# Restream/reindexer

Hardware: NVIDIA H100
Metric: KNN QPS @ recall@10 (10Mx768, k=10) + HBM GB/s vs roofline (higher is better)
Workload: dtype f32

## Files before the change

### reindexer_b200/csrc/index.cu

```cuda
#include <cuda_runtime.h>

#include <cub/device/device_scan.cuh>
#include <cub/device/device_segmented_radix_sort.cuh>

#include <algorithm>
#include <atomic>
#include <cstdio>
#include <cstdlib>
#include <cstring>
#include <limits>
#include <memory>
#include <mutex>
#include <new>
#include <string>
#include <unordered_map>
#include <unordered_set>
#include <vector>

#include "../../include/rxgpu.h"
#include "internal.h"
#include "../host/knn_select.h"
#include "knn_scan.cuh"
#include "knn_tc.cuh"
#include "ivf_select.cuh"
// ... 138 lines not shown
		a.queries = d_queries + size_t(q0) * ix->dim;
		a.nq = std::min<uint32_t>(qt, nq - q0);
		for (uint32_t round = 0; round < rounds; ++round) {
			a.k1 = std::min(kr, k1 - round * kr);
			a.floor_keys = round ? ws.d_floor.p : nullptr;
			cudaEvent_t e0 = nullptr, e1 = nullptr;
			if (g_profile.load(std::memory_order_relaxed)) {
				RX_CUDA(cudaEventCreate(&e0));
				RX_CUDA(cudaEventCreate(&e1));
				RX_CUDA(cudaEventRecord(e0, st));
			}
			RX_CUDA(launchScan(ix, qt, a, &grid, st));
			if (e0) {
				RX_CUDA(cudaEventRecord(e1, st));
				g_prof_events.emplace_back(e0, e1);
			}
			MergeArgs m{};
			m.lists = ws.d_lists.p;
			m.labels = ix->d_labels;
			m.out_dist = d_out_dist;
			m.out_idx = d_out_idx;
			m.out_label = d_out_label;
			m.out_count = d_out_count;
			m.floor_out = rounds > 1 ? ws.d_floor.p : nullptr;
			m.nlists = grid;
			m.qt = qt;
			m.k1 = a.k1;
			m.q_offset = q0;
			m.out_stride = k1;
			m.out_offset = round * kr;
			m.mode = mode;
			m.neg_zero = ix->metric != RXGPU_L2;
			knn_merge_lists<<<a.nq, 256, 0, st>>>(m);
			RX_CUDA(cudaGetLastError());
			g_stats.launches += 2;
			g_stats.passes += 1;
		}
	}
	g_stats.query_tile = uint32_t(qt);
	const uint64_t perPass = uint64_t(nrows) * ix->dim * 4 + (ix->metric == RXGPU_COS ? uint64_t(nrows) * 4 : 0) +
							 uint64_t(qt) * ix->dim * 4 + uint64_t(qt) * kr * 12;
	g_stats.algorithmic_bytes += perPass * ((nq + qt - 1) / qt) * rounds;
	return 0;
}

using EncodeTiledFn = CUresult (*)(CUtensorMap*, CUtensorMapDataType, cuuint32_t, void*, const cuuint64_t*, const cuuint64_t*,
								   const cuuint32_t*, const cuuint32_t*, CUtensorMapInterleave, CUtensorMapSwizzle, CUtensorMapL2promotion,
								   CUtensorMapFloatOOBfill);
EncodeTiledFn encodeTiled() {
	static EncodeTiledFn fn = [] {
		void* p = nullptr;
		cudaDriverEntryPointQueryResult q;
		if (cudaGetDriverEntryPoint("cuTensorMapEncodeTiled", &p, cudaEnableDefault, &q) != cudaSuccess || q != cudaDriverEntryPointSuccess) {
			cudaGetLastError();
			return EncodeTiledFn(nullptr);
		}
		return reinterpret_cast<EncodeTiledFn>(p);
	}();
	return fn;
}
int makeCodeMap(CUtensorMap* m, void* base, uint64_t pitchBytes, uint64_t rows, uint32_t boxRows) {
	const cuuint64_t gdim[2] = {pitchBytes, rows};
	const cuuint64_t gstr[1] = {pitchBytes};
	const cuuint32_t box[2] = {uint32_t(kTcChunkK), boxRows};
	const cuuint32_t estr[2] = {1, 1};
	const CUresult r = encodeTiled()(m, CU_TENSOR_MAP_DATA_TYPE_UINT8, 2, base, gdim, gstr, box, estr, CU_TENSOR_MAP_INTERLEAVE_NONE,
									  CU_TENSOR_MAP_SWIZZLE_128B, CU_TENSOR_MAP_L2_PROMOTION_L2_256B, CU_TENSOR_MAP_FLOAT_OOB_FILL_NONE);
	if (r != CUDA_SUCCESS) {
		return fail(RXGPU_ERR_SYSTEM, "rxgpu: cuTensorMapEncodeTiled failed (" + std::to_string(int(r)) + ")");
	}
	return 0;
}

constexpr size_t kTcSmemLimit = 227 * 1024;
uint32_t tcCandCap(uint32_t k1) { return std::max<uint32_t>(4096u, 256u * k1); }
uint32_t tcRangeCap(uint64_t max_out) { return uint32_t(std::max<uint64_t>(4096u, 2 * std::min<uint64_t>(max_out, 1u << 17))); }
constexpr uint32_t kStageRatio = 4;
constexpr uint32_t kStageSeedPerK1 = 2;
constexpr uint32_t kStageCapPerK1 = 64;
uint32_t stageSeedRows(uint32_t k1) { return kStageSeedPerK1 * k1; }
uint32_t stageCandCap(uint32_t k1) { return std::min<uint32_t>(1u << 18, std::max<uint32_t>(4096u, kStageCapPerK1 * k1)); }

using TcKernel = void (*)(const CUtensorMap, const TcArgs);
TcKernel tcKernel(uint32_t nqb, uint32_t cluster) {
	static const TcKernel table[4][2] = {{knn_tc_filter<32, 1>, knn_tc_filter<32, 2>},
										 {knn_tc_filter<64, 1>, knn_tc_filter<64, 2>},
										 {knn_tc_filter<96, 1>, knn_tc_filter<96, 2>},
										 {knn_tc_filter<128, 1>, knn_tc_filter<128, 2>}};
	return table[nqb / 32 - 1][cluster == 2 ? 1 : 0];
}
std::atomic<int> g_tc_diag{0};
unsigned long long* g_tc_diag_buf = nullptr;
TcKernel tcDiagKernel(int mode) {
	static const TcKernel table[4] = {knn_tc_filter<128, 1, kTcDiagStamps>, knn_tc_filter<128, 1, kTcDiagNoRare>,
									  knn_tc_filter<128, 1, kTcDiagNoFetch>, knn_tc_filter<128, 1, kTcDiagNoTest>};
	return table[mode - 1];
}

uint32_t tcQueryBlock(uint32_t nq, uint32_t kchunks) {
	uint32_t nqb = std::min<uint32_t>(kTcMaxNq, (nq + 31u) & ~31u);
	while (nqb >= 32 && tc_smem_bytes(nqb, kchunks) > kTcSmemLimit) {
		nqb -= 32;
	}
	if (nqb < 32) {
		return 0;
	}
	const uint32_t blocks = (nq + nqb - 1) / nqb;
	return std::min(nqb, (((nq + blocks - 1) / blocks) + 31u) & ~31u);
}

bool tcServes(const rxgpu_index* ix, uint32_t nq) {
	if (ix->tc_mode == 2 || !encodeTiled()) {
		return false;
	}
	if (tcQueryBlock(nq, (ix->dim + kTcChunkK - 1) / kTcChunkK) == 0) {
		return false;
	}
	if (ix->dim > 2048) {
		return false;
	}
	return ix->tc_mode == 1 || (nq >= 64 && ix->size >= 100000);
}
bool tcEligible(const rxgpu_index* ix, uint32_t nq, uint32_t k1, int mode) {
	return mode == kModeTopK && k1 <= kTcStagedMaxK1 && tcServes(ix, nq);
}

int ensureShadow(const rxgpu_index* ix, cudaStream_t st) {
	std::lock_guard<std::mutex> lck(ix->tc_mtx);
	const uint32_t pitchQ = (ix->dim + kTcChunkK - 1) / kTcChunkK * kTcChunkK;
	if (!ix->d_shadow) {
		const size_t cap = (size_t(ix->capacity ? ix->capacity : 1) + kTcTileRows - 1) / kTcTileRows * kTcTileRows;
		RX_CUDA(cudaMalloc(&ix->d_shadow, cap * pitchQ));
		RX_CUDA(cudaMalloc(reinterpret_cast<void**>(&ix->d_rowc), cap * sizeof(float4)));
		ix->pitch_q = pitchQ;
		ix->shadow_version = ~0ull;
		ix->shadow_dirty_all = true;
		ix->shadow_dirty.clear();
	}
	if (ix->shadow_version != ix->version) {
		auto convert = [&](uint32_t b, uint32_t e) {
			const unsigned blocks = unsigned((uint64_t(e - b) * 32 + 255) / 256);
			tc_convert_rows<<<blocks, 256, 0, st>>>(ix->d_rows, ix->pitch, ix->dim, b, e, static_cast<unsigned char*>(ix->d_shadow),
													pitchQ / kTcChunkK, ix->metric == RXGPU_COS ? ix->d_norms : nullptr, ix->d_rowc);
		};
		if (ix->shadow_dirty_all) {
			if (ix->size) {
				convert(0, uint32_t(ix->size));
			}
		} else {
			for (const auto& r : ix->shadow_dirty) {
				const uint32_t e = uint32_t(std::min<uint64_t>(r.second, ix->size));
				if (r.first < e) {
					convert(r.first, e);
				}
			}
		}
		ix->shadow_dirty_all = false;
		ix->shadow_dirty.clear();
		const uint64_t padded = (ix->size + kTcTileRows - 1) / kTcTileRows * kTcTileRows;
		RX_CUDA(cudaMemsetAsync(ix->d_rowc + ix->size, 0, size_t(padded - ix->size) * sizeof(float4), st));
		RX_CUDA(cudaGetLastError());
		RX_CUDA(cudaStreamSynchronize(st));
		ix->shadow_version = ix->version;
		g_stats.launches += 1;
	}
	return 0;
}

struct TcBatch {
	uint32_t nq, nqb, cluster, ngroups, nqPad, kchunks, stages, queueSlots;
	int diag;
	size_t smem;
	int resident;
	TcKernel kfn;
	CUtensorMap mapQ;
};

int tcPrepare(const rxgpu_index* ix, Workspace& ws, cudaStream_t st, const float* d_queries, uint32_t nq, uint32_t candCap, TcBatch& b) {
	if (int rc = ensureShadow(ix, st)) {
		return rc;
	}
	const uint32_t pitchQ = ix->pitch_q, kchunks = pitchQ / kTcChunkK;
	const uint32_t nqb = tcQueryBlock(nq, kchunks);
	const uint32_t ntiles = uint32_t((ix->size + kTcTileRows - 1) / kTcTileRows);
	const uint32_t clusterMax = ix->tc_cluster_max ? ix->tc_cluster_max : 1u;
	const uint32_t cluster = clusterMax >= 2 && nq > nqb && ntiles >= 2 ? 2u : 1u;
	const uint32_t ngroups = ((nq + nqb - 1) / nqb + cluster - 1) / cluster;
	const uint32_t nqPad = ngroups * cluster * nqb;
	RX_CUDA(ws.d_qcodes.ensure(size_t(nqPad) * pitchQ));
	RX_CUDA(ws.d_qc.ensure(nqPad));
	RX_CUDA(ws.d_qf.ensure(size_t(nqPad) * pitchQ));
	RX_CUDA(ws.d_tau.ensure(nqPad));
	RX_CUDA(ws.d_cand_count.ensure(nqPad));
	RX_CUDA(ws.d_cand_rows.ensure(size_t(nqPad) * candCap));
	RX_CUDA(ws.h_cand_count.ensure(nqPad));
	tc_prepare_queries<<<(nqPad * 32 + 255) / 256, 256, 0, st>>>(d_queries, nq, nqPad, ix->dim, pitchQ, ws.d_qcodes.p, ws.d_qc.p,
																 ws.d_qf.p);
	g_stats.launches += 1;
	RX_CUDA(cudaGetLastError());
	if (int rc = makeCodeMap(&b.mapQ, ws.d_qcodes.p, pitchQ, nqPad, nqb)) {
		return rc;
	}
	b.kfn = tcKernel(nqb, cluster);
	b.stages = tc_ring_stages(nqb, kchunks, kTcSmemLimit);
	b.queueSlots = tc_queue_slots(nqb, kchunks, b.stages, kTcSmemLimit);
	b.smem = tc_smem_bytes(nqb, kchunks, b.stages) + tc_queue_bytes(b.queueSlots);
	if (b.stages == 0 || b.queueSlots == 0) {
		return fail(RXGPU_ERR_SYSTEM, "rxgpu: no room for the tensor-core filter's candidate queues");
	}
	b.diag = g_tc_diag.load();
	if (const int diag = b.diag) {
		if (nqb != 128 || cluster != 1) {
			return fail(RXGPU_ERR_PARAMS, "rxgpu: the diagnostic filter instantiations take query blocks of 128 and single CTAs");
		}
		b.kfn = tcDiagKernel(diag);
	}
	RX_CUDA(raiseSmemCeilingOnce(b.kfn, ix->device, int(kTcSmemLimit)));
	cudaLaunchConfig_t cfg{};
	cfg.gridDim = dim3(unsigned(ix->sm_count) / cluster * cluster);
	cfg.blockDim = dim3(kTcThreads);
	cfg.dynamicSmemBytes = b.smem;
	cudaLaunchAttribute attr[1];
	attr[0].id = cudaLaunchAttributeClusterDimension;
	attr[0].val.clusterDim.x = cluster;
	attr[0].val.clusterDim.y = 1;
	attr[0].val.clusterDim.z = 1;
	cfg.attrs = attr;
	cfg.numAttrs = 1;
	b.resident = 0;
	RX_CUDA(cudaOccupancyMaxActiveClusters(&b.resident, b.kfn, &cfg));
	if (b.resident < 1) {
		return fail(RXGPU_ERR_SYSTEM, "rxgpu: tensor-core filter kernel cannot be made resident");
	}
	b.nq = nq;
	b.nqb = nqb;
	b.cluster = cluster;
	b.ngroups = ngroups;
	b.nqPad = nqPad;
	b.kchunks = kchunks;
	return 0;
}

int tcLaunch(const rxgpu_index* ix, Workspace& ws, cudaStream_t st, const TcBatch& b, uint32_t k1, uint32_t candCap, uint32_t nrows, bool fixedTau) {
	const uint32_t nq = b.nq, nqb = b.nqb, cluster = b.cluster, ngroups = b.ngroups, kchunks = b.kchunks, pitchQ = ix->pitch_q;
	const uint32_t ntiles = (nrows + kTcTileRows - 1) / kTcTileRows;
	const int resident = b.resident;
	const TcKernel kfn = b.kfn;
	const CUtensorMap mapQ = b.mapQ;
	RX_CUDA(cudaMemsetAsync(ws.d_cand_count.p, 0, size_t(b.nqPad) * 4, st));
	RX_CUDA(cudaGetLastError());
	cudaLaunchConfig_t cfg{};
	cfg.blockDim = dim3(kTcThreads);
	cfg.dynamicSmemBytes = b.smem;
	cfg.stream = st;
	cudaLaunchAttribute attr[1];
	attr[0].id = cudaLaunchAttributeClusterDimension;
	attr[0].val.clusterDim.x = cluster;
	attr[0].val.clusterDim.y = 1;
	attr[0].val.clusterDim.z = 1;
	cfg.attrs = attr;
	cfg.numAttrs = 1;
	TcArgs a{};
	a.shadow = static_cast<const unsigned char*>(ix->d_shadow);
	a.rowc = ix->d_rowc;
	a.qc = ws.d_qc.p;
	a.tau = ws.d_tau.p;
	a.ub_list = fixedTau ? nullptr : ws.d_ub_list.p;
	a.ub_lock = fixedTau ? nullptr : ws.d_ub_lock.p;
	a.init_rows = fixedTau ? UINT32_MAX : uint32_t(std::min<uint64_t>(ix->size, kTcInitRows));
	a.rows = ix->d_rows;
	a.norm_coefs = ix->metric == RXGPU_COS ? ix->d_norms : nullptr;
	a.qf = ws.d_qf.p;
	a.pitch = ix->pitch;
	a.cand_rows = ws.d_cand_rows.p;
	a.cand_count = ws.d_cand_count.p;
	a.cand_cap = candCap;
	a.n = nrows;
	a.dim = ix->dim;
	a.kchunks = kchunks;
	a.nq_total = nq;
	a.k1 = k1;
	a.metric = ix->metric;
	a.queue_slots = b.queueSlots;
	a.stages = b.stages;
	a.diag = g_tc_diag_buf;
	for (uint32_t g0 = 0; g0 < ngroups;) {
		const uint32_t groups = std::min<uint32_t>(ngroups - g0, uint32_t(resident));
		const uint32_t walkers = uint32_t(std::min<uint64_t>(uint32_t(resident) / groups, ntiles));
		cfg.gridDim = dim3(groups * walkers * cluster);
		a.q0 = g0 * cluster * nqb;
		a.groups = groups;
		cudaEvent_t e0 = nullptr, e1 = nullptr;
		if (g_profile.load(std::memory_order_relaxed)) {
			RX_CUDA(cudaEventCreate(&e0));
			RX_CUDA(cudaEventCreate(&e1));
			RX_CUDA(cudaEventRecord(e0, st));
		}
		RX_CUDA(cudaLaunchKernelEx(&cfg, kfn, mapQ, a));
// ... 612 lines not shown
			return fail(RXGPU_ERR_LOGIC, "The number of elements exceeds the specified limit\n");
		}
	} catch (const std::bad_alloc&) {
		return fail(RXGPU_ERR_SYSTEM, "rxgpu: out of host memory");
	}
	return 0;
}

int rxgpu_index_upsert(rxgpu_index* ix, uint64_t label, const float* vec) { return rxgpu_index_upsert_batch(ix, 1, &label, vec); }

int rxgpu_index_remove(rxgpu_index* ix, uint64_t label) {
	if (int rc = checkIndex(ix)) {
		return rc;
	}
	const uint32_t cur = ix->dict.find(label);
	if (cur == LabelMap::kNotFound) {
		return 0;
	}
	ix->dict.erase(label);
	ix->version++;
	const uint64_t last = ix->size - 1;
	if (cur != last) {
		ix->touchRows(cur, uint64_t(cur) + 1);
		const uint64_t lastLabel = ix->h_labels[last];
		ix->dict.put(lastLabel, cur);
		ix->h_labels[cur] = lastLabel;
		RX_CUDA(cudaMemcpyAsync(ix->d_rows + size_t(cur) * ix->pitch, ix->d_rows + size_t(last) * ix->pitch, ix->pitch * sizeof(float),
								cudaMemcpyDeviceToDevice, ix->stream));
		RX_CUDA(cudaMemcpyAsync(ix->d_labels + cur, ix->d_labels + last, sizeof(uint64_t), cudaMemcpyDeviceToDevice, ix->stream));
		if (ix->d_norms) {
			RX_CUDA(cudaMemcpyAsync(ix->d_norms + cur, ix->d_norms + last, sizeof(float), cudaMemcpyDeviceToDevice, ix->stream));
		}
		if (ix->flags & RXGPU_FLAG_HOST_MIRROR) {
			std::memcpy(ix->h_rows.data() + size_t(cur) * ix->dim, ix->h_rows.data() + size_t(last) * ix->dim, ix->dim * sizeof(float));
		}
		RX_CUDA(cudaStreamSynchronize(ix->stream));
	}
	ix->h_labels.pop_back();
	ix->size--;
	return 0;
}

int rxgpu_index_get(const rxgpu_index* ix, uint64_t label, const float** host_row) {
	if (!ix || !host_row) {
		return fail(RXGPU_ERR_PARAMS, "rxgpu: null handle");
	}
	const uint32_t idx = ix->dict.find(label);
	if (idx == LabelMap::kNotFound) {
		return fail(RXGPU_ERR_NOT_FOUND, "Label not found");
	}
	if (ix->flags & RXGPU_FLAG_HOST_MIRROR) {
		*host_row = ix->h_rows.data() + size_t(idx) * ix->dim;
		return 0;
	}
	RX_CUDA(cudaSetDevice(ix->device));
	g_row_scratch.resize(ix->dim);
	RX_CUDA(cudaMemcpy(g_row_scratch.data(), ix->d_rows + size_t(idx) * ix->pitch, ix->dim * sizeof(float), cudaMemcpyDeviceToHost));
	*host_row = g_row_scratch.data();
	return 0;
}

uint64_t rxgpu_index_size(const rxgpu_index* ix) { return ix ? ix->size : 0; }
uint64_t rxgpu_index_capacity(const rxgpu_index* ix) { return ix ? ix->capacity : 0; }
uint64_t rxgpu_index_element_size(const rxgpu_index* ix) { return ix ? uint64_t(ix->dim) * 4 + 8 : 0; }
uint64_t rxgpu_index_device_bytes(const rxgpu_index* ix) {
	if (!ix) {
		return 0;
	}
	const uint64_t cap = ix->capacity ? ix->capacity : 1;
	return cap * ix->pitch * 4 + cap * 8 + (ix->d_norms ? cap * 4 : 0);
}
uint32_t rxgpu_index_dim(const rxgpu_index* ix) { return ix ? ix->dim : 0; }
int rxgpu_index_metric(const rxgpu_index* ix) { return ix ? ix->metric : -1; }
int rxgpu_index_device(const rxgpu_index* ix) { return ix ? ix->device : -1; }

int rxgpu_set_query_tile(rxgpu_index* ix, uint32_t qt) {
	if (!ix) {
		return fail(RXGPU_ERR_PARAMS, "rxgpu: null handle");
	}
	ix->qt_override = qt;
	return 0;
}
int rxgpu_set_tensor_core_filter(rxgpu_index* ix, int mode) {
	if (!ix || mode < 0 || mode > 4) {
		return fail(RXGPU_ERR_PARAMS, "rxgpu: tensor-core filter mode must be 0..4");
	}
	ix->tc_mode = uint32_t(mode >= 3 ? 1 : mode);
	ix->tc_cluster_max = mode == 4 ? 2u : 0u;
	return 0;
}
int rxgpu_tc_diag(int mode, void* d_counters) {
	if (mode < 0 || mode > kTcDiagNoTest || (mode && !d_counters)) {
		return fail(RXGPU_ERR_PARAMS, "rxgpu: diagnostic filter mode must be 0..4, with a counter buffer");
	}
	const char* env = std::getenv("RXGPU_TC_DIAG");
	if (mode && !(env && std::strcmp(env, "1") == 0)) {
		return fail(RXGPU_ERR_LOGIC, "rxgpu: diagnostic filter instantiations are enabled only with RXGPU_TC_DIAG=1 in the environment");
	}
	g_tc_diag_buf = static_cast<unsigned long long*>(d_counters);
	g_tc_diag.store(mode);
	return 0;
}
int rxgpu_set_profile(int on) {
	g_profile.store(on ? 1 : 0);
	return 0;
}
void rxgpu_last_search_stats(rxgpu_search_stats* out) {
	if (out) {
		*out = g_stats;
	}
}

int rxgpu_search_knn_device(const rxgpu_index* ix, uint32_t nq, const float* d_queries, uint32_t k1, float* d_out_dist,
							uint32_t* d_out_idx, uint64_t* d_out_label, uint32_t* d_out_count, void* stream) {
	if (int rc = checkIndex(ix)) {
		return rc;
	}
	g_stats = rxgpu_search_stats{};
	if (nq == 0) {
		return 0;
	}
	if (k1 == 0 || k1 > kMaxSearchK1) {
		return fail(RXGPU_ERR_PARAMS, "rxgpu: k must be in [1, 65535]");
	}
	WsLease lease(ix);
	Workspace& ws = *lease.ws;
	cudaStream_t st = stream ? static_cast<cudaStream_t>(stream) : ix->stream;
	if (ix->size == 0) {
		RX_CUDA(cudaMemsetAsync(d_out_count, 0, nq * sizeof(uint32_t), st));
		RX_CUDA(cudaStreamSynchronize(st));
		return 0;
	}
	if (int rc = scanTopK(ix, ws, st, d_queries, nq, k1, kModeTopK, 0.f, d_out_dist, d_out_idx, d_out_label, d_out_count)) {
		return rc;
	}
	RX_CUDA(cudaStreamSynchronize(st));
	collectProfile();
	return 0;
}

int rxgpu_search_tie_rows_device(const rxgpu_index* ix, const float* d_query, float dstar, uint32_t k, float* d_out_dist,
								 uint32_t* d_out_idx, uint64_t* d_out_label, uint32_t* d_out_count, void* stream) {
	if (int rc = checkIndex(ix)) {
		return rc;
	}
	if (k == 0 || k > kMaxSearchK1) {
		return fail(RXGPU_ERR_PARAMS, "rxgpu: k must be in [1, 65535]");
	}
	WsLease lease(ix);
	cudaStream_t st = stream ? static_cast<cudaStream_t>(stream) : ix->stream;
	if (ix->size == 0) {
		RX_CUDA(cudaMemsetAsync(d_out_count, 0, sizeof(uint32_t), st));
		RX_CUDA(cudaStreamSynchronize(st));
		return 0;
	}
	if (int rc = scanTopK(ix, *lease.ws, st, d_query, 1, k, kModeTieRows, dstar, d_out_dist, d_out_idx, d_out_label, d_out_count)) {
		return rc;
	}
	RX_CUDA(cudaStreamSynchronize(st));
	g_stats.tie_replays += 1;
	return 0;
}

int rxgpu_merge_shards(uint32_t nshards, uint32_t nq, uint32_t k, uint32_t k1, const float* dist, const uint32_t* idx,
					   const uint64_t* label, const uint32_t* count, const uint64_t* shard_base, float* out_dist, uint64_t* out_gidx,
					   uint64_t* out_label, uint32_t* out_count, uint8_t* need_tie) {
	if (!dist || !idx || !label || !count || !shard_base || !out_dist || !out_gidx || !out_label || !out_count || !need_tie) {
		return fail(RXGPU_ERR_PARAMS, "rxgpu: null argument");
	}
	try {
		std::vector<Hit> all;
// ... 1484 lines not shown
```

### reindexer_b200/csrc/knn_tc.cuh

```cuda
#pragma once
#include <cuda.h>

#include <type_traits>

#include "common.cuh"
#include "knn_scan.cuh"

namespace rxgpu {

constexpr int kTcThreads = 512;
constexpr int kTcConsumers = 3;
constexpr int kTcTileRows = 128;
constexpr int kTcChunkK = 128;
constexpr int kTcStages = 12;
constexpr int kTcStagesMin = 8;
constexpr int kTcBlockBytes = 64 * kTcChunkK;
constexpr uint32_t kTcMaxNq = 128;
constexpr uint32_t kTcMaxK1 = 128;
constexpr float kTcL2Eps = 1e-5f;

struct TcArgs {
	const unsigned char* shadow;
	const float4* rowc;
	const float4* qc;
// ... 1 lines not shown
	float* ub_list;
	unsigned int* ub_lock;
	uint32_t init_rows;
	const float* rows;
	const float* norm_coefs;
	const float* qf;
	uint32_t pitch;
	uint32_t* cand_rows;
	unsigned int* cand_count;
	uint32_t cand_cap;
	uint32_t n;
	uint32_t dim;
	uint32_t kchunks;
	uint32_t nq_total;
	uint32_t q0;
	uint32_t groups;
	uint32_t k1;
	int metric;
	uint32_t queue_slots;
	uint32_t stages;
	unsigned long long* diag;
};

constexpr int kTcDiagStamps = 1;
constexpr int kTcDiagNoRare = 2;
constexpr int kTcDiagNoFetch = 3;
constexpr int kTcDiagNoTest = 4;
constexpr uint32_t kTcDiagSlots = 64;
constexpr uint32_t kTcDiagWalk = 8192;
constexpr uint32_t kTcDiagMarkEvery = 64;
enum : uint32_t {
	kTcDgFull,
	kTcDgMma,
	kTcDgDrain,
	kTcDgBar1,
	kTcDgTest,
	kTcDgAppend,
	kTcDgTurn,
	kTcDgBar2,
	kTcDgTile,
	kTcDgBlocks,
	kTcDgHits,
	kTcDgQueueWait,
	kTcDgPerWg,
	kTcDgEmpty = kTcConsumers * kTcDgPerWg,
	kTcDgProd = kTcDgEmpty + 1,
	kTcDgRescored = kTcDgProd + 1,
	kTcDgInserts,
	kTcDgRescoreCycles,
};
static_assert(kTcDgRescoreCycles < kTcDiagSlots, "diagnostic counters fit their slots");

__host__ __device__ inline size_t tc_smem_bytes(uint32_t nq_block, uint32_t kchunks, uint32_t stages = kTcStages) {
	return 1024  + size_t(nq_block) * kchunks * 128 + size_t(stages) * kTcBlockBytes + 256  +
		   size_t(nq_block) * (16  + kTcConsumers * (4 + 8) ) + 64;
}

__device__ __forceinline__ uint32_t smem_u32(const void* p) { return uint32_t(__cvta_generic_to_shared(p)); }
__device__ __forceinline__ void mbar_init(uint64_t* bar, uint32_t count) {
	asm volatile("mbarrier.init.shared::cta.b64 [%0], %1;" ::"r"(smem_u32(bar)), "r"(count));
}
__device__ __forceinline__ void mbar_expect_tx(uint64_t* bar, uint32_t bytes) {
	asm volatile("mbarrier.arrive.expect_tx.shared::cta.b64 _, [%0], %1;" ::"r"(smem_u32(bar)), "r"(bytes) : "memory");
}
__device__ __forceinline__ void mbar_arrive(uint64_t* bar) {
	asm volatile("mbarrier.arrive.shared::cta.b64 _, [%0];" ::"r"(smem_u32(bar)) : "memory");
}
__device__ __forceinline__ void mbar_wait(uint64_t* bar, uint32_t parity) {
	asm volatile(
		"{\n"
		".reg .pred p;\n"
		"WAIT_%=:\n"
		"mbarrier.try_wait.parity.shared::cta.b64 p, [%0], %1;\n"
		"@p bra DONE_%=;\n"
		"bra WAIT_%=;\n"
		"DONE_%=:\n"
		"}\n" ::"r"(smem_u32(bar)),
		"r"(parity)
		: "memory");
}
__device__ __forceinline__ void mbar_arrive_cluster(uint64_t* bar, uint32_t cta) {
	uint32_t remote;
	asm volatile("mapa.shared::cluster.u32 %0, %1, %2;" : "=r"(remote) : "r"(smem_u32(bar)), "r"(cta));
	asm volatile("mbarrier.arrive.release.cluster.shared::cluster.b64 _, [%0];" ::"r"(remote) : "memory");
}
__device__ __forceinline__ void tma_load_2d(void* dst, const CUtensorMap* map, uint64_t* bar, int32_t x, int32_t y) {
	asm volatile("cp.async.bulk.tensor.2d.shared::cluster.global.tile.mbarrier::complete_tx::bytes [%0], [%1, {%3, %4}], [%2];" ::"r"(
					 smem_u32(dst)),
				 "l"(map), "r"(smem_u32(bar)), "r"(x), "r"(y)
				 : "memory");
}
__device__ __forceinline__ void bulk_load(void* dst, const void* src, uint32_t bytes, uint64_t* bar) {
	asm volatile("cp.async.bulk.shared::cluster.global.mbarrier::complete_tx::bytes [%0], [%1], %2, [%3];" ::"r"(smem_u32(dst)), "l"(src),
				 "r"(bytes), "r"(smem_u32(bar))
				 : "memory");
}
__device__ __forceinline__ void bulk_load_mc(void* dst, const void* src, uint32_t bytes, uint64_t* bar, uint16_t mask) {
	asm volatile("cp.async.bulk.shared::cluster.global.mbarrier::complete_tx::bytes.multicast::cluster [%0], [%1], %2, [%3], %4;" ::"r"(
					 smem_u32(dst)),
				 "l"(src), "r"(bytes), "r"(smem_u32(bar)), "h"(mask)
				 : "memory");
}
__device__ __forceinline__ bool elect_one_sync() {
	uint32_t p;
	asm volatile(
		"{\n"
		".reg .pred P;\n"
		"elect.sync _|P, 0xffffffff;\n"
		"selp.u32 %0, 1, 0, P;\n"
		"}\n"
		: "=r"(p));
	return p != 0;
}
__device__ __forceinline__ uint32_t cluster_ctarank() {
	uint32_t r;
	asm volatile("mov.u32 %0, %%cluster_ctarank;" : "=r"(r));
	return r;
}
__device__ __forceinline__ void cluster_sync_all() {
	asm volatile("barrier.cluster.arrive.release.aligned;" ::: "memory");
	asm volatile("barrier.cluster.wait.acquire.aligned;" ::: "memory");
}
__device__ __forceinline__ uint64_t wgmma_desc_sw128(uint32_t smem_addr) {
	uint64_t d = 0;
	d |= uint64_t((smem_addr & 0x3FFFFu) >> 4);
	d |= uint64_t(1) << 16;
	d |= uint64_t(1024 >> 4) << 32;
	d |= uint64_t(1) << 62;
	return d;
}
__device__ __forceinline__ void wgmma_fence() { asm volatile("wgmma.fence.sync.aligned;" ::: "memory"); }
__device__ __forceinline__ void wgmma_commit() { asm volatile("wgmma.commit_group.sync.aligned;" ::: "memory"); }
template <int N>
__device__ __forceinline__ void wgmma_wait() {
	asm volatile("wgmma.wait_group.sync.aligned %0;" ::"n"(N) : "memory");
}
__device__ __forceinline__ void wgmma_m64n32k32(int (&d)[16], uint64_t adesc, uint64_t bdesc, uint32_t accumulate) {
	asm volatile(
		"{\n"
		".reg .pred p;\n"
		"setp.ne.b32 p, %18, 0;\n"
		"wgmma.mma_async.sync.aligned.m64n32k32.s32.s8.s8 "
		"{%0,%1,%2,%3,%4,%5,%6,%7,%8,%9,%10,%11,%12,%13,%14,%15}, "
		"%16, %17, p;\n"
		"}\n"
		: "+r"(d[0]), "+r"(d[1]), "+r"(d[2]), "+r"(d[3]), "+r"(d[4]), "+r"(d[5]), "+r"(d[6]), "+r"(d[7]), "+r"(d[8]), "+r"(d[9]), "+r"(d[10]), "+r"(d[11]),
		  "+r"(d[12]), "+r"(d[13]), "+r"(d[14]), "+r"(d[15])
		: "l"(adesc), "l"(bdesc), "r"(accumulate));
}
__device__ __forceinline__ void wgmma_m64n64k32(int (&d)[32], uint64_t adesc, uint64_t bdesc, uint32_t accumulate) {
	asm volatile(
		"{\n"
		".reg .pred p;\n"
		"setp.ne.b32 p, %34, 0;\n"
		"wgmma.mma_async.sync.aligned.m64n64k32.s32.s8.s8 "
		"{%0,%1,%2,%3,%4,%5,%6,%7,%8,%9,%10,%11,%12,%13,%14,%15,"
		"%16,%17,%18,%19,%20,%21,%22,%23,%24,%25,%26,%27,%28,%29,%30,%31}, "
		"%32, %33, p;\n"
		"}\n"
		: "+r"(d[0]), "+r"(d[1]), "+r"(d[2]), "+r"(d[3]), "+r"(d[4]), "+r"(d[5]), "+r"(d[6]), "+r"(d[7]), "+r"(d[8]), "+r"(d[9]), "+r"(d[10]), "+r"(d[11]),
		  "+r"(d[12]), "+r"(d[13]), "+r"(d[14]), "+r"(d[15]), "+r"(d[16]), "+r"(d[17]), "+r"(d[18]), "+r"(d[19]), "+r"(d[20]), "+r"(d[21]), "+r"(d[22]), "+r"(d[23]),
		  "+r"(d[24]), "+r"(d[25]), "+r"(d[26]), "+r"(d[27]), "+r"(d[28]), "+r"(d[29]), "+r"(d[30]), "+r"(d[31])
		: "l"(adesc), "l"(bdesc), "r"(accumulate));
}
__device__ __forceinline__ void wgmma_m64n96k32(int (&d)[48], uint64_t adesc, uint64_t bdesc, uint32_t accumulate) {
	asm volatile(
		"{\n"
// ... 208 lines not shown
			}
			__nanosleep(256);
			continue;
		}
		const bool active = uint32_t(lane) < n;
		uint32_t ql = 0, row = 0;
		float x = 0.f;
		if (active) {
			const uint32_t t = head + lane;
			const uint4* r = rec + (t & (slots - 1));
			while (ld_acquire_shared(&r->w) != t + 1) {
			}
			ql = r->x;
			row = r->y;
			x = __uint_as_float(r->z);
		}
		__syncwarp();
		head += n;
		if (lane == 0) {
			st_release_shared(&qu->head, head);
		}
		float d = 0.f, err = 0.f, tau = 0.f;
		if (active) {
			const float4 qc = s_qc[ql], rc = a.rowc[row];
			const float2 de = tc_row_bound(a, x, qc, rc);
			d = de.x;
			err = de.y;
			tau = tc_min_thr<kNq>(s_thr, ql);
		}
		const bool append = active && !(d - err > tau);
		const unsigned peers = __match_any_sync(0xffffffffu, append ? ql : ~0u);
		const int leader = __ffs(peers) - 1;
		unsigned base = 0;
		if (append && lane == leader) {
			base = atomicAdd(&a.cand_count[q0 + ql], unsigned(__popc(peers)));
		}
		base = __shfl_sync(0xffffffffu, base, leader);
		if (append) {
			const unsigned pos = base + __popc(peers & ((1u << lane) - 1u));
			if (pos < a.cand_cap) {
				a.cand_rows[size_t(q0 + ql) * a.cand_cap + pos] = row;
			}
		}
		const bool rescore = append && row >= a.init_rows && d < tau;
		const unsigned todo = __ballot_sync(0xffffffffu, rescore);
		if (todo) {
			[[maybe_unused]] const long long c0 = kDiag == kTcDiagStamps ? clock64() : 0ll;
			const float dx = a.metric == kL2 ? tc_rescore<true>(a, todo, row, ql, q0, lane) : tc_rescore<false>(a, todo, row, ql, q0, lane);
			if constexpr (kDiag != 0) {
				n_rescored += __popc(todo);
				if constexpr (kDiag == kTcDiagStamps) {
					rescore_cycles += clock64() - c0;
				}
			}
			if (rescore && dx < tc_min_thr<kNq>(s_thr, ql)) {
				if constexpr (kDiag != 0) {
					++n_inserts;
				}
				const float nt = tc_bound_insert(a, q0 + ql, dx);
				for (uint32_t w = 0; w < kTcConsumers; ++w) {
					if (nt < s_thr[w * kNq + ql]) {
						s_thr[w * kNq + ql] = nt;
						s_pr[w * kNq + ql] = tc_make_pr(a.metric, nt, s_qc[ql], l2eps);
					}
				}
			}
		}
		__syncwarp();
	}
	if constexpr (kDiag != 0) {
		const unsigned long long ins = __reduce_add_sync(0xffffffffu, uint32_t(n_inserts));
		if (lane == 0) {
			atomicAdd(&dg[kTcDgRescored], n_rescored);
			atomicAdd(&dg[kTcDgInserts], ins);
			atomicAdd(&dg[kTcDgRescoreCycles], (unsigned long long)rescore_cycles);
		}
	}
}

template <int kNq, int kCluster, int kDiag = 0>
__global__ void __launch_bounds__(kTcThreads, 1)
	knn_tc_filter(const __grid_constant__ CUtensorMap map_queries, const __grid_constant__ TcArgs a) {
	static_assert(kNq % 32 == 0 && kNq <= int(kTcMaxNq), "query block");
	static_assert(kCluster == 1 || kCluster == 2, "a stage is split in 1 or 2 equal copies");
	static_assert(kDiag == 0 || kCluster == 1, "the diagnostic instantiations are single CTAs");
	constexpr bool kStamp = kDiag == kTcDiagStamps;
	auto clk = [] {
		if constexpr (kStamp) {
			return clock64();
		} else {
			return 0ll;
		}
	};
	unsigned long long* dg = kDiag ? a.diag + size_t(blockIdx.x) * kTcDiagSlots : nullptr;
	extern __shared__ unsigned char smem_raw[];
	unsigned char* base = smem_raw + ((1024u - (smem_u32(smem_raw) & 1023u)) & 1023u);
	constexpr uint32_t kQchunkBytes = kNq * 128;
	unsigned char* s_q = base;
	unsigned char* s_rows = s_q + size_t(a.kchunks) * kQchunkBytes;
	const uint32_t nstages = a.stages;
	uint64_t* bars = reinterpret_cast<uint64_t*>(s_rows + size_t(nstages) * kTcBlockBytes);
	uint64_t* full_bar = bars;
	uint64_t* empty_bar = bars + kTcStages;
	uint64_t* q_bar = bars + 2 * kTcStages;
	float* s_ab = reinterpret_cast<float*>(q_bar + 1);
	float4* s_qc = reinterpret_cast<float4*>(bars + 32);
	float* s_thr = reinterpret_cast<float*>(s_qc + kNq);
	float2* s_pr = reinterpret_cast<float2*>(s_thr + kTcConsumers * kNq);
	TcQueue* s_queue = reinterpret_cast<TcQueue*>(s_pr + kTcConsumers * kNq);
	uint4* s_rec = reinterpret_cast<uint4*>(s_queue + kTcConsumers);
	static_assert(2 * kTcStages + 2 <= 32, "barriers and (a*, b*) fit in front of the per-query constants");

	const int warp = __shfl_sync(0xffffffffu, int(threadIdx.x >> 5), 0), lane = threadIdx.x & 31;
	const uint32_t ntiles = (a.n + kTcTileRows - 1) / kTcTileRows;
	const uint32_t crank = kCluster > 1 ? cluster_ctarank() : 0u;
	const uint32_t cid = blockIdx.x / kCluster, ncl = gridDim.x / kCluster;
	const uint32_t walker = cid / a.groups, walkers = ncl / a.groups;
	const uint32_t q0 = a.q0 + ((cid % a.groups) * kCluster + crank) * kNq;
	const uint32_t nq_valid = q0 < a.nq_total ? min(uint32_t(kNq), a.nq_total - q0) : 0u;
	const float l2eps = tc_l2eps(a.dim);

	if (threadIdx.x == 0) {
		for (uint32_t s = 0; s < nstages; ++s) {
			mbar_init(&full_bar[s], 1);
			mbar_init(&empty_bar[s], 4 * kCluster);
		}
		mbar_init(q_bar, 1);
		asm volatile("fence.mbarrier_init.release.cluster;" ::: "memory");
		s_ab[0] = s_ab[1] = 0.f;
		for (int w = 0; w < kTcConsumers; ++w) {
			s_queue[w] = TcQueue{0u, 0u, 0u, 0u};
		}
	}
	for (uint32_t i = threadIdx.x; i < kTcConsumers * a.queue_slots; i += blockDim.x) {
		s_rec[i].w = 0u;
	}
	if constexpr (kDiag == kTcDiagNoFetch) {
		for (uint32_t i = threadIdx.x; i < nstages * kTcBlockBytes / 16; i += blockDim.x) {
			reinterpret_cast<uint4*>(s_rows)[i] = make_uint4(0u, 0u, 0u, 0u);
		}
		asm volatile("fence.proxy.async.shared::cta;" ::: "memory");
	}
	__syncthreads();
	const float delta = float(a.dim + 16) * 0x1p-23f;
	for (uint32_t i = threadIdx.x; i < kNq; i += blockDim.x) {
		const bool valid = i < nq_valid;
		const float thr = valid ? ord_float(a.tau[q0 + i]) : -INFINITY;
		const float4 qc = valid ? a.qc[q0 + i] : make_float4(0.f, 0.f, 0.f, 0.f);
		if (qc.z > 0.f) {
			atomicMax(reinterpret_cast<unsigned int*>(&s_ab[0]), __float_as_uint((qc.z + qc.y) / qc.z));
			atomicMax(reinterpret_cast<unsigned int*>(&s_ab[1]), __float_as_uint(qc.y / qc.z + delta));
		}
		s_qc[i] = qc;
		const float2 pr = valid ? tc_make_pr(a.metric, thr, qc, l2eps) : make_float2(0.f, -INFINITY);
		for (int w = 0; w < kTcConsumers; ++w) {
			s_thr[w * kNq + i] = thr;
			s_pr[w * kNq + i] = pr;
		}
	}
	__syncthreads();
	if constexpr (kCluster > 1) {
		cluster_sync_all();
	}
	const uint32_t nblocks = walker < ntiles ? 2 * ((ntiles - walker + walkers - 1) / walkers) : 0u;

	if (warp == 0) {
		if (elect_one_sync()) {
			mbar_expect_tx(q_bar, a.kchunks * kQchunkBytes);
			for (uint32_t kc = 0; kc < a.kchunks; ++kc) {
				tma_load_2d(s_q + size_t(kc) * kQchunkBytes, &map_queries, q_bar, int32_t(kc * kTcChunkK), int32_t(q0));
			}
		}
		__syncwarp();
		uint64_t* full = full_bar;
		uint64_t* empty = empty_bar;
		unsigned char* ring_smem = s_rows;
		uint32_t stage = 0, phase = 0;
		[[maybe_unused]] long long t_empty = 0;
		[[maybe_unused]] const long long t_start = clk();
		for (uint32_t i = 0; i < nblocks; ++i) {
			const unsigned char* src = a.shadow + size_t(2 * (walker + (i >> 1) * walkers) + (i & 1u)) * a.kchunks * kTcBlockBytes;
			for (uint32_t kc = 0; kc < a.kchunks; ++kc) {
				[[maybe_unused]] const long long c0 = clk();
				mbar_wait(&empty[stage], phase ^ 1);
				if constexpr (kStamp) {
					t_empty += clk() - c0;
				}
				unsigned char* dst = ring_smem + size_t(stage) * kTcBlockBytes;
				if constexpr (kDiag == kTcDiagNoFetch) {
					if (elect_one_sync()) {
						mbar_arrive(&full[stage]);
					}
				} else if (elect_one_sync()) {
					mbar_expect_tx(&full[stage], kTcBlockBytes);
					if constexpr (kCluster == 1) {
						bulk_load(dst, src + size_t(kc) * kTcBlockBytes, kTcBlockBytes, &full[stage]);
					} else {
						constexpr uint32_t kPart = kTcBlockBytes / kCluster;
						bulk_load_mc(dst + crank * kPart, src + size_t(kc) * kTcBlockBytes + crank * kPart, kPart, &full[stage],
									 uint16_t((1u << kCluster) - 1u));
					}
				}
				__syncwarp();
				if (++stage == nstages) {
					stage = 0;
					phase ^= 1;
				}
			}
		}
		if constexpr (kStamp) {
			if (lane == 0) {
				atomicAdd(&dg[kTcDgEmpty], (unsigned long long)t_empty);
				atomicAdd(&dg[kTcDgProd], (unsigned long long)(clk() - t_start));
			}
		}
	} else if (warp < 4) {
		const uint32_t wg = uint32_t(warp) - 1;
		tc_bookkeeper<kNq, kDiag>(a, s_queue + wg, s_rec + wg * a.queue_slots, a.queue_slots, q0, s_qc, s_thr, s_pr, l2eps, lane, dg);
	} else {
		const uint32_t wg = uint32_t(warp) / 4 - 1, wtid = threadIdx.x - 128 * (wg + 1);
		float* thr = s_thr + wg * kNq;
		float2* pr = s_pr + wg * kNq;
		TcQueue* qu = s_queue + wg;
		uint4* rec = s_rec + wg * a.queue_slots;
		const uint32_t slots = a.queue_slots;
		uint64_t* full = full_bar;
		uint64_t* empty = empty_bar;
		const unsigned char* ring_smem = s_rows;
		const uint32_t r0 = (wtid >> 5) * 16 + (lane >> 2), c2 = 2 * (lane & 3);
		const uint32_t my_q = wtid;
		unsigned int tau_ahead = my_q < nq_valid ? a.tau[q0 + my_q] : 0u;
		const bool l2 = a.metric == kL2;
		const float ka = (1.f + 0x1p-7f) * s_ab[0], kb = (1.f + 0x1p-7f) * s_ab[1];
		auto release = [&](uint32_t st) {
			if constexpr (kCluster == 1) {
				mbar_arrive(&empty[st]);
			} else {
				for (uint32_t c = 0; c < uint32_t(kCluster); ++c) {
					mbar_arrive_cluster(&empty[st], c);
				}
			}
		};
		mbar_wait(q_bar, 0);
		[[maybe_unused]] long long dt[kTcDgPerWg] = {};
		[[maybe_unused]] unsigned long long nhits = 0;
		[[maybe_unused]] uint32_t sink = 0;
		for (uint32_t blk = wg; blk < nblocks; blk += kTcConsumers) {
			const uint32_t t = walker + (blk >> 1) * walkers, half = blk & 1u;
			[[maybe_unused]] const uint32_t walk = blk >> 1;
			[[maybe_unused]] long long s0 = clk(), s1, s2, s3, s4, s5;
			if constexpr (kStamp) {
				if (half == 0 && wtid == 0 && walk % kTcDiagMarkEvery == 0 && walk < kTcDiagWalk) {
					unsigned long long now;
					asm volatile("mov.u64 %0, %%globaltimer;" : "=l"(now));
					a.diag[size_t(gridDim.x) * kTcDiagSlots + kTcDiagWalk + size_t(blockIdx.x) * (kTcDiagWalk / kTcDiagMarkEvery) +
						   walk / kTcDiagMarkEvery] = now;
				}
			}
			if (my_q < nq_valid) {
				const float tn = ord_float(tau_ahead);
				if (tn < thr[my_q]) {
					thr[my_q] = tn;
					pr[my_q] = tc_make_pr(a.metric, tn, s_qc[my_q], l2eps);
				}
				tau_ahead = a.tau[q0 + my_q];
			}
			const uint32_t row0 = (2 * t + half) * 64 + r0, row1 = row0 + 8;
			const float4 rc0 = a.rowc[row0], rc1 = a.rowc[row1];
			int acc[kNq / 2];
#pragma unroll
			for (int i = 0; i < kNq / 2; ++i) {
				acc[i] = 0;
			}
			const uint32_t g0 = blk * a.kchunks;
			uint32_t stage = g0 % nstages, phase = (g0 / nstages) & 1u;
			[[maybe_unused]] const long long c_turn = clk();
			if (blk != 0) {
				asm volatile("bar.sync %0, 256;" ::"r"(4 + wg) : "memory");
			}
			if constexpr (kStamp) {
				dt[kTcDgTurn] += clk() - c_turn;
			}
			uint32_t prev = 0;
			for (uint32_t kc = 0; kc < a.kchunks; ++kc) {
				[[maybe_unused]] const long long c0 = clk();
				mbar_wait(&full[stage], phase);
				if constexpr (kStamp) {
					dt[kTcDgFull] += clk() - c0;
				}
				const uint32_t a_addr = smem_u32(ring_smem + size_t(stage) * kTcBlockBytes);
				const uint32_t b_addr = smem_u32(s_q + size_t(kc) * kQchunkBytes);
				wgmma_fence();
#pragma unroll
				for (uint32_t k = 0; k < kTcChunkK / 32; ++k) {
					wgmma_s8<kNq>(acc, wgmma_desc_sw128(a_addr + k * 32), wgmma_desc_sw128(b_addr + k * 32), (kc | k) != 0);
				}
				wgmma_commit();
				if (kc > 0) {
					wgmma_wait<1>();
					if (lane == 0) {
						release(prev);
					}
				}
				prev = stage;
				if (++stage == nstages) {
					stage = 0;
					phase ^= 1;
				}
			}
			if (blk + 1 < nblocks) {
				asm volatile("bar.arrive %0, 256;" ::"r"(4 + (wg + 1) % kTcConsumers) : "memory");
			}
			s1 = clk();
			wgmma_wait<0>();
			if (lane == 0) {
				release(prev);
			}
			s2 = clk();
			asm volatile("bar.sync %0, 128;" ::"r"(1 + wg) : "memory");
			s3 = clk();
			const float S0 = rc0.x * rc0.w, S1 = rc1.x * rc1.w;
			const float M0 = rc0.w * fmaf(ka, rc0.y, kb * rc0.z), M1 = rc1.w * fmaf(ka, rc1.y, kb * rc1.z);
			const float W0 = l2 ? 0.5f * (1.f - l2eps) * rc0.z * rc0.z : 0.f, W1 = l2 ? 0.5f * (1.f - l2eps) * rc1.z * rc1.z : 0.f;
			const uint32_t ok = (row0 < a.n ? 0x33333333u : 0u) | (row1 < a.n ? 0xCCCCCCCCu : 0u);
			constexpr int kMaskWords = (kNq / 2 + 31) / 32;
			uint32_t hm[kMaskWords] = {};
			auto test = [&](auto kL2Tag) {
				constexpr bool kL2 = decltype(kL2Tag)::value;
#pragma unroll
				for (int j = 0; j < kNq / 8; ++j) {
					const uint32_t q = 8 * j + c2;
					const float4 p2 = *reinterpret_cast<const float4*>(&pr[q]);
					float Ra = p2.y, Rb = p2.w, Rc = p2.y, Rd = p2.w;
					if constexpr (kL2) {
						const float za = s_qc[q].w, zb = s_qc[q + 1].w;
						Ra = fmaf(-za, W0, Ra);
						Rb = fmaf(-zb, W0, Rb);
						Rc = fmaf(-za, W1, Rc);
						Rd = fmaf(-zb, W1, Rd);
					}
					const float x0 = float(acc[4 * j]), x1 = float(acc[4 * j + 1]), x2 = float(acc[4 * j + 2]), x3 = float(acc[4 * j + 3]);
					const bool h0 = !(fmaf(x0, S0, fmaf(p2.x, M0, Ra)) < 0.f);
					const bool h1 = !(fmaf(x1, S0, fmaf(p2.z, M0, Rb)) < 0.f);
					const bool h2 = !(fmaf(x2, S1, fmaf(p2.x, M1, Rc)) < 0.f);
					const bool h3 = !(fmaf(x3, S1, fmaf(p2.z, M1, Rd)) < 0.f);
					hm[4 * j / 32] |= (uint32_t(h0) | uint32_t(h1) << 1 | uint32_t(h2) << 2 | uint32_t(h3) << 3) << (4 * j % 32);
				}
			};
			if constexpr (kDiag == kTcDiagNoTest) {
#pragma unroll
				for (int i = 0; i < kNq / 2; ++i) {
					sink ^= uint32_t(acc[i]);
				}
			} else if (l2) {
				test(std::true_type{});
			} else {
				test(std::false_type{});
			}
#pragma unroll
			for (int w = 0; w < kMaskWords; ++w) {
				hm[w] &= ok;
			}
			s4 = clk();
			[[maybe_unused]] uint32_t nh = 0;
#pragma unroll
			for (int w = 0; w < kMaskWords; ++w) {
				nh += __popc(hm[w]);
			}
			if constexpr (kDiag != 0) {
				nhits += nh;
			}
			if constexpr (kDiag != kTcDiagNoRare && kDiag != kTcDiagNoTest) {
				if (__any_sync(0xffffffffu, nh != 0)) {
#pragma unroll
					for (int j = 0; j < kNq / 8; ++j) {
						const uint32_t h = hm[4 * j / 32] >> (4 * j % 32) & 15u;
						if (h) {
							const bool waited = tc_enqueue_quad(qu, rec, slots, h, 8 * j + c2, row0, row1, float(acc[4 * j]), float(acc[4 * j + 1]),
																float(acc[4 * j + 2]), float(acc[4 * j + 3]));
							if constexpr (kStamp) {
								if (waited) {
									atomicAdd(&qu->full_waits, 1u);
								}
							}
						}
					}
				}
			}
			__syncwarp();
			s5 = clk();
			asm volatile("bar.sync %0, 128;" ::"r"(1 + wg) : "memory");
			if constexpr (kStamp) {
				const long long s6 = clk();
				dt[kTcDgMma] += s1 - s0;
				dt[kTcDgDrain] += s2 - s1;
				dt[kTcDgBar1] += s3 - s2;
				dt[kTcDgTest] += s4 - s3;
				dt[kTcDgAppend] += s5 - s4;
				dt[kTcDgBar2] += s6 - s5;
				dt[kTcDgTile] += s6 - s0;
// ... 468 lines not shown
```

Baseline: 67140.

## Enable thread-block clusters by default for large indexes and add 4-CTA clusters

Adds 4-CTA cluster instantiations of the tensor-core filter and picks the cluster size from the number of query blocks, with little padding allowed. Indexes of at least 8M rows now default to 2-CTA clusters, so one TMA multicast of database tiles serves several query blocks and cuts HBM traffic per query. The remote empty-barrier arrivals are spread across lanes instead of run serially by lane 0, and the release ordering qualifier on the cluster arrive is dropped. Risks are cluster scheduling limits, query-block padding waste, and a weaker memory-ordering guarantee on the slot release.

```diff
diff --git a/reindexer_b200/csrc/index.cu b/reindexer_b200/csrc/index.cu
--- a/reindexer_b200/csrc/index.cu
+++ b/reindexer_b200/csrc/index.cu
@@ -244,19 +244,24 @@
 uint32_t stageCandCap(uint32_t k1) { return std::min<uint32_t>(1u << 18, std::max<uint32_t>(4096u, kStageCapPerK1 * k1)); }
 
 using TcKernel = void (*)(const CUtensorMap, const TcArgs);
+int tcClusterIndex(uint32_t cluster) { return cluster == 4 ? 2 : cluster == 2 ? 1 : 0; }
 TcKernel tcKernel(uint32_t nqb, uint32_t cluster) {
-	static const TcKernel table[4][2] = {{knn_tc_filter<32, 1>, knn_tc_filter<32, 2>},
-										 {knn_tc_filter<64, 1>, knn_tc_filter<64, 2>},
-										 {knn_tc_filter<96, 1>, knn_tc_filter<96, 2>},
-										 {knn_tc_filter<128, 1>, knn_tc_filter<128, 2>}};
-	return table[nqb / 32 - 1][cluster == 2 ? 1 : 0];
+	static const TcKernel table[4][3] = {{knn_tc_filter<32, 1>, knn_tc_filter<32, 2>, knn_tc_filter<32, 4>},
+										 {knn_tc_filter<64, 1>, knn_tc_filter<64, 2>, knn_tc_filter<64, 4>},
+										 {knn_tc_filter<96, 1>, knn_tc_filter<96, 2>, knn_tc_filter<96, 4>},
+										 {knn_tc_filter<128, 1>, knn_tc_filter<128, 2>, knn_tc_filter<128, 4>}};
+	return table[nqb / 32 - 1][tcClusterIndex(cluster)];
 }
 std::atomic<int> g_tc_diag{0};
 unsigned long long* g_tc_diag_buf = nullptr;
-TcKernel tcDiagKernel(int mode) {
-	static const TcKernel table[4] = {knn_tc_filter<128, 1, kTcDiagStamps>, knn_tc_filter<128, 1, kTcDiagNoRare>,
-									  knn_tc_filter<128, 1, kTcDiagNoFetch>, knn_tc_filter<128, 1, kTcDiagNoTest>};
+template <int kCluster>
+TcKernel tcDiagKernelC(int mode) {
+	static const TcKernel table[4] = {knn_tc_filter<128, kCluster, kTcDiagStamps>, knn_tc_filter<128, kCluster, kTcDiagNoRare>,
+									  knn_tc_filter<128, kCluster, kTcDiagNoFetch>, knn_tc_filter<128, kCluster, kTcDiagNoTest>};
 	return table[mode - 1];
+}
+TcKernel tcDiagKernel(int mode, uint32_t cluster) {
+	return cluster == 4 ? tcDiagKernelC<4>(mode) : cluster == 2 ? tcDiagKernelC<2>(mode) : tcDiagKernelC<1>(mode);
 }
 
 uint32_t tcQueryBlock(uint32_t nq, uint32_t kchunks) {
@@ -329,6 +334,18 @@
 	return 0;
 }
 
+constexpr uint32_t kTcClusterDefault = 2;
+constexpr uint64_t kTcClusterMinRows = 1u << 23;
+uint32_t tcClusterSize(uint32_t nblocks, uint32_t ntiles, uint32_t cmax) {
+	for (uint32_t c = cmax; c > 1; c /= 2) {
+		const uint32_t pad = (c - nblocks % c) % c;
+		if (ntiles >= 2 && pad <= 1 && pad < nblocks) {
+			return c;
+		}
+	}
+	return 1;
+}
+
 struct TcBatch {
 	uint32_t nq, nqb, cluster, ngroups, nqPad, kchunks, stages, queueSlots;
 	int diag;
@@ -345,9 +362,10 @@
 	const uint32_t pitchQ = ix->pitch_q, kchunks = pitchQ / kTcChunkK;
 	const uint32_t nqb = tcQueryBlock(nq, kchunks);
 	const uint32_t ntiles = uint32_t((ix->size + kTcTileRows - 1) / kTcTileRows);
-	const uint32_t clusterMax = ix->tc_cluster_max ? ix->tc_cluster_max : 1u;
-	const uint32_t cluster = clusterMax >= 2 && nq > nqb && ntiles >= 2 ? 2u : 1u;
-	const uint32_t ngroups = ((nq + nqb - 1) / nqb + cluster - 1) / cluster;
+	const uint32_t nblocks = (nq + nqb - 1) / nqb;
+	const uint32_t cmax = ix->tc_cluster_max ? ix->tc_cluster_max : ix->size >= kTcClusterMinRows ? kTcClusterDefault : 1u;
+	const uint32_t cluster = tcClusterSize(nblocks, ntiles, cmax);
+	const uint32_t ngroups = (nblocks + cluster - 1) / cluster;
 	const uint32_t nqPad = ngroups * cluster * nqb;
 	RX_CUDA(ws.d_qcodes.ensure(size_t(nqPad) * pitchQ));
 	RX_CUDA(ws.d_qc.ensure(nqPad));
@@ -372,10 +390,10 @@
 	}
 	b.diag = g_tc_diag.load();
 	if (const int diag = b.diag) {
-		if (nqb != 128 || cluster != 1) {
-			return fail(RXGPU_ERR_PARAMS, "rxgpu: the diagnostic filter instantiations take query blocks of 128 and single CTAs");
-		}
-		b.kfn = tcDiagKernel(diag);
+		if (nqb != 128) {
+			return fail(RXGPU_ERR_PARAMS, "rxgpu: the diagnostic filter instantiations take query blocks of 128");
+		}
+		b.kfn = tcDiagKernel(diag, cluster);
 	}
 	RX_CUDA(raiseSmemCeilingOnce(b.kfn, ix->device, int(kTcSmemLimit)));
 	cudaLaunchConfig_t cfg{};
@@ -1154,11 +1172,11 @@
 	return 0;
 }
 int rxgpu_set_tensor_core_filter(rxgpu_index* ix, int mode) {
-	if (!ix || mode < 0 || mode > 4) {
-		return fail(RXGPU_ERR_PARAMS, "rxgpu: tensor-core filter mode must be 0..4");
+	if (!ix || mode < 0 || mode > 5) {
+		return fail(RXGPU_ERR_PARAMS, "rxgpu: tensor-core filter mode must be 0..5");
 	}
 	ix->tc_mode = uint32_t(mode >= 3 ? 1 : mode);
-	ix->tc_cluster_max = mode == 4 ? 2u : 0u;
+	ix->tc_cluster_max = mode == 3 ? 1u : mode == 4 ? 2u : mode == 5 ? 4u : 0u;
 	return 0;
 }
 int rxgpu_tc_diag(int mode, void* d_counters) {
diff --git a/reindexer_b200/csrc/knn_tc.cuh b/reindexer_b200/csrc/knn_tc.cuh
--- a/reindexer_b200/csrc/knn_tc.cuh
+++ b/reindexer_b200/csrc/knn_tc.cuh
@@ -107,7 +107,7 @@
 __device__ __forceinline__ void mbar_arrive_cluster(uint64_t* bar, uint32_t cta) {
 	uint32_t remote;
 	asm volatile("mapa.shared::cluster.u32 %0, %1, %2;" : "=r"(remote) : "r"(smem_u32(bar)), "r"(cta));
-	asm volatile("mbarrier.arrive.release.cluster.shared::cluster.b64 _, [%0];" ::"r"(remote) : "memory");
+	asm volatile("mbarrier.arrive.shared::cluster.b64 _, [%0];" ::"r"(remote) : "memory");
 }
 __device__ __forceinline__ void tma_load_2d(void* dst, const CUtensorMap* map, uint64_t* bar, int32_t x, int32_t y) {
 	asm volatile("cp.async.bulk.tensor.2d.shared::cluster.global.tile.mbarrier::complete_tx::bytes [%0], [%1, {%3, %4}], [%2];" ::"r"(
@@ -482,8 +482,7 @@
 __global__ void __launch_bounds__(kTcThreads, 1)
 	knn_tc_filter(const __grid_constant__ CUtensorMap map_queries, const __grid_constant__ TcArgs a) {
 	static_assert(kNq % 32 == 0 && kNq <= int(kTcMaxNq), "query block");
-	static_assert(kCluster == 1 || kCluster == 2, "a stage is split in 1 or 2 equal copies");
-	static_assert(kDiag == 0 || kCluster == 1, "the diagnostic instantiations are single CTAs");
+	static_assert(kCluster == 1 || kCluster == 2 || kCluster == 4, "a stage is split in 1, 2 or 4 equal copies");
 	constexpr bool kStamp = kDiag == kTcDiagStamps;
 	auto clk = [] {
 		if constexpr (kStamp) {
@@ -634,11 +633,11 @@
 		const float ka = (1.f + 0x1p-7f) * s_ab[0], kb = (1.f + 0x1p-7f) * s_ab[1];
 		auto release = [&](uint32_t st) {
 			if constexpr (kCluster == 1) {
-				mbar_arrive(&empty[st]);
-			} else {
-				for (uint32_t c = 0; c < uint32_t(kCluster); ++c) {
-					mbar_arrive_cluster(&empty[st], c);
-				}
+				if (lane == 0) {
+					mbar_arrive(&empty[st]);
+				}
+			} else if (lane < kCluster) {
+				mbar_arrive_cluster(&empty[st], uint32_t(lane));
 			}
 		};
 		mbar_wait(q_bar, 0);
@@ -698,9 +697,7 @@
 				wgmma_commit();
 				if (kc > 0) {
 					wgmma_wait<1>();
-					if (lane == 0) {
-						release(prev);
-					}
+					release(prev);
 				}
 				prev = stage;
 				if (++stage == nstages) {
@@ -713,9 +710,7 @@
 			}
 			s1 = clk();
 			wgmma_wait<0>();
-			if (lane == 0) {
-				release(prev);
-			}
+			release(prev);
 			s2 = clk();
 			asm volatile("bar.sync %0, 128;" ::"r"(1 + wg) : "memory");
 			s3 = clk();
```

Result: faster. 69880 (median of 6 runs) (+4.1%).
